# fryzjergda/DesiRNA

Hardware: AMD Instinct MI355X
Metric: replica-folds/sec (MFE+PF, L=200, R=64) (higher is better)
Workload: dtype int32 (MFE) + f64 (PF); 1 GPU; BASELINE configs[2]: Eterna100-V1 #69 target (L=200), R=64 uniform-random sequences per GPU, -sf Ed-Epf (MFE fill+traceback, PF inside, eval_structure); replicas_per_gpu=64, replicas_total=64, replicas_on_rank0=64, L=200, exchange_every=100, threads_per_workgroup=1024

## Files before the change

desirna_amd/csrc/engine.hip:

```cpp
#include <hip/hip_runtime.h>

#include <cstdio>
#include <cstdlib>
#include <cstring>
#include <ctime>
#include <algorithm>
#include <numeric>
#include <string>
#include <vector>

#include "../../include/desirna_amd.h"
#include "eval_structure.hpp"
#include "fold_mfe.hpp"
#include "fold_cofold.hpp"
#include "fold_cofold_lds.hpp"
#include "fold_self_dimer.hpp"
#include "fold_mfe_lds.hpp"
#include "fold_mfe_dual.hpp"
#include "fold_fused.hpp"
#include "fold_mfe_strip.hpp"
#include "fold_outside.hpp"
#include "fold_pf.hpp"
#include "fold_pf_lds.hpp"
#include "fold_pf_strip.hpp"
// ... 582 lines not shown
  else if (p.mfe_strips && ma.pk_rounds > 0 && R >= 16 * e->mfe_split && e->mfe_split > 1) {
    const int np = e->mfe_split, per = ((R + np - 1) / np + 7) / 8 * 8;
    const int pf_gate_round = pf_gate_env >= -1 ? pf_gate_env : (p.pf_strips && p.mfe_wgs >= e->cus && ma.pk_rounds >= 2) ? ma.pk_rounds - 1 : -1;
    for (int round = 0; round <= ma.pk_rounds; round++) {
      for (int part = 0, r0 = 0; r0 < R; part++, r0 += per) {
        const bool gate_here = round == pf_gate_round && p.want_pf && part == pf_gate_part;
        launch_mfe_strips_round(e, ma, std::min(per, R - r0), p.mfe_strips, r0, nullptr, r0, (part & 1) ? e->s_eval : e->s_mfe, round,
                                gate_here ? e->ev_gate : nullptr);
        if (gate_here) c.pf_gated = true;
      }
    }
    HIP_TRY(hipEventRecord(e->ev_mfe2, e->s_eval));
    HIP_TRY(hipStreamWaitEvent(e->s_mfe, e->ev_mfe2, 0));
  } else if (p.mfe_strips) launch_mfe_strips(e, ma, R, p.mfe_strips, 0, nullptr, e->s_mfe);
  else if (c.L <= MFE_FAST_NMAX) hipLaunchKernelGGL(mfe_lds_kernel<1024>, dim3(R), dim3(1024), 0, e->s_mfe, ma);
  else hipLaunchKernelGGL(mfe_kernel<1024>, dim3(R), dim3(1024), 0, e->s_mfe, ma);
  HIP_TRY(hipGetLastError());
  HIP_TRY(hipEventRecord(e->ev_m1, e->s_mfe));
  return DRNA_OK;
}
static int enqueue_eval(drna_engine* e, const FoldCall& c) {
  if (c.p.ev_in_pf) return DRNA_OK;
  HIP_TRY(hipEventRecord(e->ev_e0, c.s_ev));
  hipLaunchKernelGGL(eval_kernel, dim3(c.R * e->n_targets), dim3(WAVE), 0, c.s_ev, c.ev);
  HIP_TRY(hipGetLastError());
  HIP_TRY(hipEventRecord(e->ev_e1, c.s_ev));
  return DRNA_OK;
}
static int enqueue_folds(drna_engine* e, FoldCall& c) {
  const FoldPlan& p = c.p;
  e->last_fused = p.fused;
  e->last_wgs = p.mfe_wgs + p.pf_wgs;
  if (p.fused) {
    HIP_TRY(hipEventRecord(e->ev_m0, e->s_mfe));
    hipLaunchKernelGGL(score_fused_kernel<1024>, dim3(fused_grid(c.R)), dim3(1024), 0, e->s_mfe, c.ma, c.lk, c.pa, c.ev, c.R, e->d_clk);
    HIP_TRY(hipGetLastError());
    HIP_TRY(hipEventRecord(e->ev_m1, e->s_mfe));
    return DRNA_OK;
  }
  c.mfe_first = p.want_mfe && (!p.want_pf || e->timing[0] > e->timing[1]);
  c.s_ev = !(p.want_mfe && p.want_pf) ? e->s_eval : c.mfe_first ? e->s_pf : e->s_mfe;
  if (c.mfe_first) { const int rc = enqueue_mfe(e, c); if (rc != DRNA_OK) return rc; }
  if (p.want_ev && c.s_ev == e->s_pf) { const int rc = enqueue_eval(e, c); if (rc != DRNA_OK) return rc; }
  if (p.want_pf) { const int rc = enqueue_pf(e, c); if (rc != DRNA_OK) return rc; }
  if (p.want_ev && c.s_ev == e->s_mfe) { const int rc = enqueue_eval(e, c); if (rc != DRNA_OK) return rc; }
  if (p.want_mfe && !c.mfe_first) { const int rc = enqueue_mfe(e, c); if (rc != DRNA_OK) return rc; }
  if (p.want_ev && c.s_ev == e->s_eval) { const int rc = enqueue_eval(e, c); if (rc != DRNA_OK) return rc; }
  return DRNA_OK;
}

static int drain_folds(drna_engine* e, const FoldCall& c) {
  const FoldPlan& p = c.p;
  if (p.fused) {
    HIP_TRY(hipStreamSynchronize(e->s_mfe));
    float tot = 0.f;
    HIP_TRY(hipEventElapsedTime(&tot, e->ev_m0, e->ev_m1));
    const int grid = fused_grid(c.R);
    long long t0 = 0, end_mfe = 0, end_pf = 0;
    bool first = true;
    for (int b = 0; b < grid; b++) {
      int r, role;
      fused_block_role(b, r, role, grid);
      if (r >= c.R) continue;
      const long long s0 = e->h_clk[2 * b], s1 = e->h_clk[2 * b + 1];
      if (first || s0 < t0) t0 = s0;
      first = false;
      if (role <= ROLE_MFE_HELPER) { if (s1 > end_mfe) end_mfe = s1; } else if (s1 > end_pf) end_pf = s1;
    }
    e->timing[0] = (float)((end_mfe - t0) * 1e-5); e->timing[1] = (float)((end_pf - t0) * 1e-5);
    e->timing[2] = 0.f; e->timing[3] = tot;
    return DRNA_OK;
  }
  const bool ev_own = p.want_ev && !p.ev_in_pf;
  if (ev_own && c.s_ev == e->s_eval) HIP_TRY(hipStreamSynchronize(e->s_eval));
  if (c.mfe_first && p.want_pf) HIP_TRY(hipStreamSynchronize(e->s_pf));
  if (p.want_mfe) HIP_TRY(hipStreamSynchronize(e->s_mfe));
  if (!c.mfe_first && p.want_pf) HIP_TRY(hipStreamSynchronize(e->s_pf));
  e->timing[0] = e->timing[1] = e->timing[2] = e->timing[3] = 0.f;
  if (p.want_mfe) HIP_TRY(hipEventElapsedTime(&e->timing[0], e->ev_m0, e->ev_m1));
  if (p.want_pf) HIP_TRY(hipEventElapsedTime(&e->timing[1], e->ev_p0, e->ev_p1));
  if (ev_own) HIP_TRY(hipEventElapsedTime(&e->timing[2], e->ev_e0, e->ev_e1));
  hipEvent_t first = c.mfe_first ? e->ev_m0 : p.want_pf ? e->ev_p0 : e->ev_e0;
  float t = 0.f;
  if (p.want_mfe) { HIP_TRY(hipEventElapsedTime(&t, first, e->ev_m1)); e->timing[3] = std::max(e->timing[3], t); }
  if (p.want_pf) { HIP_TRY(hipEventElapsedTime(&t, first, e->ev_p1)); e->timing[3] = std::max(e->timing[3], t); }
  if (ev_own) { HIP_TRY(hipEventElapsedTime(&t, first, e->ev_e1)); e->timing[3] = std::max(e->timing[3], t); }
  return DRNA_OK;
}

static int score_batch_impl(drna_engine* e, int R, int L, const char* d_seqs, uint32_t flags, double* d_Epf, int32_t* d_Emfe,
                            char* d_mfe_ss, int32_t* d_Ed, int r_base) {
  HIP_TRY(hipSetDevice(e->device));
  FoldCall c{R, L, plan_uniform(e, R, L, flags)};
  const FoldPlan& p = c.p;
  { const int rc = prepare_folds(e, p, R); if (rc != DRNA_OK) return rc; }
  reset_status(e);
  e->cur_with_pf = p.want_pf;
  c.ev = p.want_ev ? eval_args(e, d_seqs, L, d_Ed) : EvalArgs{};
  c.ma = mfe_args(e, d_seqs, L, L + 2, p.want_pk ? 3 : 0, d_Emfe, d_mfe_ss);
  c.pa = pf_args(e, d_seqs, L, L + 2, d_Epf);
  if (p.pf_help) { c.pa.helper = e->helper_fault ? 2 : 1; c.pa.hflags = e->pflags.d; c.pa.hbase = epoch_base(e->pflags.epoch); }
  c.lk.flagA = e->dflags.d; c.lk.flagB = e->dflags.d;
  c.lk.xs = e->d_xs; c.lk.xa = e->d_xa_mfe; c.lk.xb = e->d_xb_mfe; c.lk.epoch = e->dflags.epoch;
// ... 1728 lines not shown
```

desirna_amd/csrc/fold_mfe.hpp:

```cpp
#pragma once
#include "fold_common.hpp"

namespace drna {

struct MfeArgs {
  const MfeTables* T;
  const Plan* plan;
  const int* hp_len;
  const char* seqs;
  int L;
  int ld;
  int pk_rounds;
  int32_t* ws;
  long long ws_stride;
  int32_t* Emfe;
  char* ss;
  int32_t* status;
  Ragged rg;
};

template <int NLEN>
struct MfeSmemCore {
  int stack[64];
  int mmH[128], mmI[128], mm1n[128], mm23[128], mmM[128], mmExt[128];
// ... 287 lines not shown
      }
      m = wave_min_i32(m);
      const int prev = sm.f5[j - 1];
      sm.f5[j] = prev < m ? prev : m;
    }
  }
  __syncthreads();
}


struct FmlGlobal {
  const int32_t* p;
  int ld;
  __device__ __forceinline__ int operator()(int d, int i) const { return p[d * ld + i]; }
};

template <class SM> struct TbStack {
  SM& sm;
  int sp = 0;
  __device__ __forceinline__ void init(int n) { sm.sec_i[0] = 1; sm.sec_j[0] = (short)n; sm.sec_ml[0] = 0; sp = 1; }
  __device__ __forceinline__ bool pop(int& i, int& j, int& ml) {
    if (sp == 0) return false;
    sp--;
    i = sm.sec_i[sp]; j = sm.sec_j[sp]; ml = sm.sec_ml[sp];
    return true;
  }
  __device__ __forceinline__ void push(int i, int j, int ml) { sm.sec_i[sp] = (short)i; sm.sec_j[sp] = (short)j; sm.sec_ml[sp] = (unsigned char)ml; sp++; }
  __device__ __forceinline__ void done_one() {}
  __device__ __forceinline__ void fail() {}
  __device__ __forceinline__ bool failed() const { return false; }
};
template <class SM> struct TbShared {
  SM& sm;
  __device__ __forceinline__ void init(int) {}
  __device__ __forceinline__ bool pop(int& i, int& j, int& ml) {
    int c = 0;
    if (lane_id() == 0) c = atomicAdd(&sm.tbq[0], 1);
    c = __builtin_amdgcn_readfirstlane(c);
    if (c > (int)(sizeof(sm.sec_ml) / sizeof(sm.sec_ml[0])) - 1) return false;
    for (;;) {
      const int m = __builtin_amdgcn_readfirstlane((int)*reinterpret_cast<volatile unsigned char*>(&sm.sec_ml[c]));
      if (m) {
        __builtin_amdgcn_fence(__ATOMIC_ACQUIRE, "workgroup");
        i = sm.sec_i[c]; j = sm.sec_j[c]; ml = m - 1;
        return true;
      }
      if (__builtin_amdgcn_readfirstlane(*reinterpret_cast<volatile int*>(&sm.tbq[3]))) return false;
      spin_pause();
    }
  }
  __device__ __forceinline__ void push(int i, int j, int ml) {
    if (lane_id() == 0) {
      atomicAdd(&sm.tbq[2], 1);
      const int c = atomicAdd(&sm.tbq[1], 1);
      if (c > (int)(sizeof(sm.sec_ml) / sizeof(sm.sec_ml[0])) - 1) { *reinterpret_cast<volatile int*>(&sm.tbq[3]) = 2; return; }
      sm.sec_i[c] = (short)i; sm.sec_j[c] = (short)j;
      __builtin_amdgcn_fence(__ATOMIC_RELEASE, "workgroup");
      *reinterpret_cast<volatile unsigned char*>(&sm.sec_ml[c]) = (unsigned char)(ml + 1);
    }
  }
  __device__ __forceinline__ void done_one() {
    if (lane_id() == 0 && atomicAdd(&sm.tbq[2], -1) == 1) *reinterpret_cast<volatile int*>(&sm.tbq[3]) = 1;
  }
  __device__ __forceinline__ void fail() { if (lane_id() == 0) *reinterpret_cast<volatile int*>(&sm.tbq[3]) = 2; }
  __device__ __forceinline__ bool failed() const { return *reinterpret_cast<volatile int*>(&sm.tbq[3]) == 2; }
};

template <class SM, class FMLACC, class QUEUE>
__device__ __forceinline__ bool mfe_traceback_q(SM& sm, const MfeArgs& A, const int32_t* __restrict__ Wc,
                                       const FMLACC FML, const int32_t* __restrict__ EXT, QUEUE Q) {
  const MfeTables& T = *A.T;
  const Plan& P = *A.plan;
  const int n = A.L, ld = A.ld, lane = lane_id();
  const int HALF = INF_DEV / 2;
  bool ok = true;
  constexpr int NRND = (NPLAN + WAVE - 1) / WAVE;
  int tb_shape[NRND], tb_L[NRND];
#pragma unroll
  for (int rnd = 0; rnd < NRND; rnd++) {
    const int k = rnd * WAVE + lane;
    tb_shape[rnd] = k < NPLAN ? P.tb_shape[k] : (PK_STACK << 16);
    tb_L[rnd] = k < NPLAN ? P.tb_L[k] : 0;
  }
  Q.init(n);
  auto sector = [&](int i, int j, const int ml) -> bool {
    bool have_pair = false;
    if (ml == 0) {
      if (j < TURN + 2) return true;
      int jj = -1;
      for (int base = j; base >= 1 && jj < 0; base -= WAVE) {
        const int x = base - lane;
        const bool hit = x >= 1 && sm.f5[x] != sm.f5[x - 1];
        const int fl = first_lane(__ballot(hit));
        if (fl >= 0) jj = base - fl;
      }
      if (jj < TURN + 2) return true;
      const int fij = sm.f5[jj];
      int u = -1;
      for (int base = jj - TURN - 1; base >= 1 && u < 0; base -= WAVE) {
        const int x = base - lane;
        bool hit = false;
        if (x >= 1) {
          const int e = EXT[jj * ld + x];
          hit = e < HALF && fij == e + sm.f5[x - 1];
        }
        const int fl = first_lane(__ballot(hit));
        if (fl >= 0) u = base - fl;
      }
      if (u < 0) return false;
      Q.push(1, (u - 1), 0);
      i = u; j = jj; have_pair = true;
    } else if (ml == 1) {
      for (;;) {
        const int jx = j - lane;
        bool stop = true;
        if (jx > i) {
          const int a = FML(jx - i, i), bq = (jx - 1 - i) >= 0 ? FML(jx - 1 - i, i) : INF_DEV;
          stop = !(a == bq + T.MLbase);
        }
        const int fl = first_lane(__ballot(stop));
        if (fl >= 0) { j -= fl; break; }
        j -= WAVE;
      }
      for (;;) {
        const int ix = i + lane;
        bool stop = true;
        if (ix < j) {
          const int a = FML(j - ix, ix), bq = FML(j - ix - 1, ix + 1);
          stop = !(a == bq + T.MLbase);
        }
        const int fl = first_lane(__ballot(stop));
        if (fl >= 0) { i += fl; break; }
        i += WAVE;
      }
      if (j < i + TURN + 1) return false;
      const int d = j - i;
      const int fij = FML(d, i);
      const int w = Wc[d * ld + i];
      const int cij = w >> 8;
      const int t = pair_type(sm.Sp[i], sm.Sp[j]);
      if (t && cij < HALF &&
          fij == cij + T.MLintern + (t > 2 ? T.TermAU : 0) + sm.mmM[t * 16 + sm.S[i - 1] * 4 + sm.S[j + 1]]) {
        have_pair = true;
      } else {
        int u = -1;
        for (int base = i + TURN + 1; base <= j - TURN - 2 && u < 0; base += WAVE) {
          const int x = base + lane;
          bool hit = false;
          if (x <= j - TURN - 2) hit = fij == FML(x - i, i) + FML(j - x - 1, x + 1);
          const int fl = first_lane(__ballot(hit));
          if (fl >= 0) u = base + fl;
        }
        if (u < 0) return false;
        Q.push(i, u, 1);
        Q.push((u + 1), j, 1);
      }
    } else {
      have_pair = true;
    }
    while (have_pair) {
      if (lane == 0) { sm.ssw[i - 1] = '('; sm.ssw[j - 1] = ')'; }
      const int d = j - i;
      const int t = pair_type(sm.Sp[i], sm.Sp[j]);
      const int w_in = d - 2 > TURN ? Wc[(d - 2) * ld + i + 1] : INF_DEV * 256;
      const int cij = Wc[d * ld + i] >> 8;
      if (cij == mfe_hairpin(sm, A, i, j, t)) break;
      const int si1 = sm.S[i + 1], sj1 = sm.S[j - 1];
      if ((w_in >> 8) < HALF && cij == (w_in >> 8) + mfe_intloop(sm, T, 0, 0, t, si1, sj1, w_in & 127)) {
        i++; j--;
        continue;
      }
      int found = -1;
      const int tij = t * 16 + si1 * 4 + sj1, tauI = t > 2 ? T.TermAU : 0;
#pragma unroll
      for (int rnd = 0; rnd < NRND; rnd++) {
        if (found >= 0) break;
        const int k = rnd * WAVE + lane;
        const int u1 = tb_shape[rnd] & 255, u2 = (tb_shape[rnd] >> 8) & 255, kind = tb_shape[rnd] >> 16;
        const int dp = d - 2 - u1 - u2;
        const bool live = k < NPLAN && dp > TURN;
        const int w = live ? Wc[dp * ld + i + 1 + u1] : INF_DEV * 256;
        const int cpq = w >> 8, info = w & 127, t2 = info >> 4, sq1 = (info >> 2) & 3, sp1 = info & 3;
        const int* mm = kind == PK_1XN ? sm.mm1n : kind == PK_INT23 ? sm.mm23 : sm.mmI;
        int en = mm[tij] + mm[info];
        const int e_stack = sm.stack[t * 8 + t2], e_11 = sm.int11[(t * 8 + t2) * 16 + si1 * 4 + sj1];
        en = kind == PK_STACK || kind == PK_BULGE1 ? e_stack : en;
        en = kind == PK_BULGEN ? tauI + (t2 > 2 ? T.TermAU : 0) : en;
        en = kind == PK_INT11 ? e_11 : en;
        if (kind == PK_INT21) en = T.int21[(t * 8 + t2) * 64 + si1 * 16 + sq1 * 4 + sj1];
        else if (kind == PK_INT12) en = T.int21[(t2 * 8 + t) * 64 + sq1 * 16 + si1 * 4 + sp1];
        else if (kind == PK_INT22) en = T.int22[(t * 8 + t2) * 256 + si1 * 64 + sp1 * 16 + sq1 * 4 + sj1];
        const bool hit = live && cpq < HALF && cij == cpq + en + tb_L[rnd];
        const int fl = first_lane(__ballot(hit));
        if (fl >= 0) found = rnd * WAVE + fl;
      }
      if (found >= 0) {
        i = i + 1 + P.tb_u1[found];
        j = j - 1 - P.tb_u2[found];
        continue;
      }
      const int e = cij - T.MLclosing - T.MLintern - (t > 2 ? T.TermAU : 0) -
                    sm.mmM[rtype_of(t) * 16 + sj1 * 4 + si1];
      int u = -1;
      for (int base = i + 2 + TURN; base < j - 2 - TURN && u < 0; base += WAVE) {
        const int x = base + lane;
        bool hit = false;
        if (x < j - 2 - TURN) hit = e == FML(x - i - 1, i + 1) + FML(j - 1 - x - 1, x + 1);
        const int fl = first_lane(__ballot(hit));
        if (fl >= 0) u = base + fl;
      }
      if (u < 0) return false;
      Q.push((i + 1), u, 1);
      Q.push((u + 1), (j - 1), 1);
      break;
    }
    return true;
  };
  int qi = 0, qj = 0, qml = 0;
  while (Q.pop(qi, qj, qml)) {
    if (!sector(qi, qj, qml)) { Q.fail(); ok = false; break; }
    Q.done_one();
  }
  return ok && !Q.failed();
}

template <class SM, class FMLACC>
__device__ inline bool mfe_traceback(SM& sm, const MfeArgs& A, const int32_t* __restrict__ Wc,
                                     const FMLACC FML, const int32_t* __restrict__ EXT) {
  return mfe_traceback_q(sm, A, Wc, FML, EXT, TbStack<SM>{sm});
}



template <int NT>
__global__ __launch_bounds__(NT) void mfe_kernel(MfeArgs A) {
  __shared__ MfeSmem sm;
  const int r = A.rg.seq_of(blockIdx.x);
  A.L = A.rg.len_of(r, A.L);
  const long long so = A.rg.off_of(r, A.L);
  const int n = A.L, ld = A.ld, tid = threadIdx.x;
  const MfeTables& T = *A.T;
  int32_t* base = A.ws + (long long)r * A.ws_stride;
  const long long tab = (long long)ld * ld;
  int32_t* Wc = base;
  int32_t* CI = base + tab;
  int32_t* FML = base + 2 * tab;
  int32_t* DML = base + 3 * tab;
  int32_t* EXT = base + 4 * tab;

  stage_energy_tables<NT>(sm, T, tid);
  load_sequence<NT>(sm, A.seqs + so, n, tid);
  if (sm.flag) {
    if (tid == 0) { A.status[r] = ST_BAD_CHAR; A.Emfe[r] = 0; }
    for (int k = tid; k < n; k += NT) A.ss[so + k] = '.';
    return;
  }
  pk_start<NT>(sm, n, tid);

  int status = ST_OK;
  for (int round = 0; round <= A.pk_rounds; round++) {
    for (int k = tid; k < n; k += NT) sm.ssw[k] = '.';
    mfe_fill<NT>(sm, A, Wc, CI, FML, DML, EXT);
// ... 17 lines not shown
```

desirna_amd/csrc/fold_mfe_lds.hpp:

```cpp
#pragma once
#include "fold_mfe.hpp"

namespace drna {

constexpr int MFE_FAST_NMAX = 200;
enum : int { E_ALL = 0, E_NEAR = 1, E_FAR = 2, E_COARSE = 3 };
constexpr int GSLOTS = 10;

template <int NT>
struct MfeFastSmem : MfeSmemCore<MFE_FAST_NMAX> {
  static constexpr int NW = NT / WAVE;
  static constexpr int RS = MFE_FAST_NMAX + 2;
  static constexpr int TRI = (MFE_FAST_NMAX - 4) * (MFE_FAST_NMAX - 3) / 2;
  static constexpr int NSLOT = 4 * WAVE;
  static constexpr int NL = MFE_FAST_NMAX + 8;
  int fml[TRI + 8];
  int wring[33 * RS];
  int ciring[32 * RS];
  int dml[4 * RS];
  int hpl[MFE_FAST_NMAX + 2];
  int rowoff[MFE_FAST_NMAX + 2];
  int accG[2][NSLOT], accI[2][NSLOT], accK[2][NSLOT];
  static constexpr int XT_STACK = 0, XT_INT11 = 64, XT_MM1N = 64 + 1024, XT_MM23 = 64 + 1024 + 128;
  int xtab[64 + 1024 + 128 + 128];
  int plist[2][NL];
  int xe[2][NL];
  int pcnt[2];
  int qhead[2];
  int eshape[128];
  int eshape_rows[128];
  int sync_fail;
  int tbq[4];
  int etab[2][128];
  int twc[32][2];
};

__device__ __forceinline__ int fml_off(int d, int n) { return (d - 4) * n - (d * (d - 1) / 2 - 6); }

template <int NT>
struct FmlLds {
  const MfeFastSmem<NT>* sm;
  int n;
  __device__ __forceinline__ int operator()(int d, int i) const {
    return d < TURN + 1 ? INF_DEV : sm->fml[fml_off(d, n) + i - 1];
  }
};

template <int NT>
__device__ __forceinline__ void mfe_f5_column(MfeFastSmem<NT>& sm, const int32_t* __restrict__ EXT, int ld, int j, int lane) {
  int m = INF_DEV;
  for (int i = lane + 1; i <= j - TURN - 1; i += WAVE) {
    const int x = EXT[j * ld + i];
    if (x < INF_DEV / 2) m = min(m, sm.f5[i - 1] + x);
  }
  m = wave_min_i32(m);
  const int prev = sm.f5[j - 1];
  sm.f5[j] = prev < m ? prev : m;
}

template <class SM>
__device__ __forceinline__ void mfe_prepare_etab(SM& sm, int d, int lane, int mode);
template <class SM>
__device__ __forceinline__ void mfe_prepare_tower_tab(SM& sm, int d, int tid, int ninio, int max_ninio) {
  constexpr int RS = SM::RS;
  const int par = d & 1;
// ... 744 lines not shown
  const long long so = A.rg.off_of(r, A.L);
  const int n = A.L, ld = A.ld, tid = threadIdx.x;
  const MfeTables& T = *A.T;
  int32_t* base = A.ws + (long long)r * A.ws_stride;
  const long long tab = (long long)ld * ld;
  int32_t* Wc = base;
  int32_t* EXT = base + 4 * tab;
  int32_t* PL = base + 3 * tab;
  int32_t* PLX = base + 1 * tab;

  for (int k = tid; k < 64; k += NT) sm.stack[k] = T.stack[k];
  for (int k = tid; k < 128; k += NT) {
    sm.mmH[k] = T.mmH[k]; sm.mmI[k] = T.mmI[k]; sm.mm1n[k] = T.mm1n[k];
    sm.mm23[k] = T.mm23[k]; sm.mmM[k] = T.mmM[k]; sm.mmExt[k] = T.mmExt[k];
  }
  for (int k = tid; k < 1024; k += NT) sm.int11[k] = T.int11[k];
  for (int k = tid; k < 32; k += NT) { sm.d5[k] = T.d5[k]; sm.d3[k] = T.d3[k]; }
  if (tid == 0) sm.sync_fail = 0;
  load_sequence<NT>(sm, A.seqs + so, n, tid);
  if (sm.flag) {
    if (tid == 0) { A.status[r] = ST_BAD_CHAR; A.Emfe[r] = 0; if (DUAL) st_agent(lk.flagA, dual_done(lk.epoch)); }
    for (int k = tid; k < n; k += NT) A.ss[so + k] = '.';
    return;
  }
  pk_start<NT>(sm, n, tid);

  int status = ST_OK;
  for (int round = 0; round <= A.pk_rounds; round++) {
    for (int k = tid; k < n; k += NT) sm.ssw[k] = '.';
    lk.base = dual_base(lk.epoch, round);
    mfe_fill_lds<NT, DUAL>(sm, A, Wc, EXT, PL, PLX, lk);
    if (DUAL && sm.sync_fail) { status = ST_SYNC; break; }
    constexpr int TB_WAVES = NT / WAVE < 8 ? NT / WAVE : 8;
    for (int k = tid; k < (int)(sizeof(sm.sec_ml) / sizeof(sm.sec_ml[0])); k += NT) sm.sec_ml[k] = 0;
    __syncthreads();
    if (tid == 0) {
      sm.sec_i[0] = 1; sm.sec_j[0] = (short)n; sm.sec_ml[0] = 1;
      sm.tbq[0] = 0; sm.tbq[1] = 1; sm.tbq[2] = 1; sm.tbq[3] = 0;
    }
    __syncthreads();
    if (wave_id() < TB_WAVES) (void)mfe_traceback_q(sm, A, Wc, FmlLds<NT>{&sm, n}, EXT, TbShared<MfeFastSmem<NT>>{sm});
    __syncthreads();
    if (tid == 0) {
      if (round == 0) A.Emfe[r] = sm.f5[n];
      sm.flag = sm.tbq[3] == 2 ? 1 : 0;
    }
    __syncthreads();
    if (sm.flag) { status = ST_TRACEBACK; break; }
    if (!pk_merge_round<NT>(sm, n, round)) break;
  }
  if (DUAL && tid == 0) st_agent(lk.flagA, dual_done(lk.epoch));
  for (int k = tid; k < n; k += NT) A.ss[so + k] = sm.sspk[k];
  if (tid == 0) A.status[r] = status;
}

template <int NT>
__global__ __launch_bounds__(NT) void mfe_lds_kernel(MfeArgs A) {
  __shared__ MfeFastSmem<NT> sm;
  const int r = A.rg.seq_of(blockIdx.x);
  mfe_lds_body<NT, false>(sm, A, r, DualLink{});
}

}
```

desirna_amd/csrc/fold_mfe_strip.hpp:

```cpp
#pragma once
#include "fold_mfe_lds.hpp"
#include <type_traits>

namespace drna {

constexpr int MSTRIP_REC = 96;

constexpr int MSTRIP_KU = 8;
#ifndef DRNA_MKT_W
#define DRNA_MKT_W 16
#endif
#ifndef DRNA_MKT_L
#define DRNA_MKT_L 4
#endif
constexpr int MKT_W = DRNA_MKT_W, MKT_L = DRNA_MKT_L;
constexpr int MKT_DEPTH = 2;
constexpr int MKT_BMIN = (44 + 2 * MKT_L + 15) / 16;
static_assert(MKT_W >= 1 && MKT_W <= 16 && MKT_L >= 3, "see tools/pkt_schedule.py");

template <int N>
__device__ __forceinline__ int row_bcast_i32(int v) { return __builtin_amdgcn_update_dpp(0, v, 0x150 + N, 0xF, 0xF, false); }

template <int NT>
struct MfeStripSmem {
// ... 618 lines not shown
  if (failed) {
    if (tid == 0) {
      if (has_down) st_agent(my_flag, lk.base + STRIP_FAIL);
      else { A.status[r] = ST_SYNC; Wc[0] = -1; }
    }
    return;
  }
  if (lk.clk && tid == 0) lk.clk[((long long)q * STRIP_MAXS + s) * 2 + 1] = wall_clock_100mhz();
  if (has_down) {
    if (tid == 0) st_agent(my_flag, lk.base + STRIP_DONE);
    return;
  }
  if (wave == 0) {
    for (int j = max(TURN + 2, n - 2); j <= n; j++) mstrip_f5_column(sm, rsE, ld, j, lane);
  }
  __syncthreads();
  for (int k = tid; k <= n; k += NT) Wc[ld + k] = sm.f5[k];
  if (tid == 0) Wc[0] = 2;
}

template <int NT, bool FARK>
__global__ __launch_bounds__(NT) void mfe_strip_kernel(MfeArgs A, StripLink lk, StripRec xr, int round) {
  __shared__ MfeStripSmem<NT> sm;
  const int b = blockIdx.x, per = 8 * (lk.S + lk.pad);
  const int grp = b / per, x = b - grp * per;
  const int q = grp * 8 + (x & 7), s = x >> 3;
  if (q >= lk.nseq || s >= lk.S) return;
  mfe_strip_body<NT, FARK>(sm, A, lk, xr, q, s, round);
}

constexpr int TRACE_WAVES = 8;
struct MfeTraceSmem : MfeSmemCore<STRIP_NMAX> {
  int tbq[4];
};

__device__ inline void mfe_strip_trace_body(MfeTraceSmem& sm, MfeArgs A, const int* idx, int q, int round, int r0 = 0) {
  constexpr int NT = TRACE_WAVES * WAVE;
  const int r = idx ? idx[q] : q + r0;
  A.L = A.rg.len_of(r, A.L);
  const long long so = A.rg.off_of(r, A.L);
  const int n = A.L, ld = A.ld, tid = threadIdx.x;
  const MfeTables& T = *A.T;
  int32_t* base = A.ws + (long long)r * A.ws_stride;
  const long long tab = (long long)ld * ld;
  int32_t* Wc = base;
  const int32_t* FML = base + 2 * tab;
  const int32_t* EXT = base + 4 * tab;
  const int state = Wc[0];
  if (round > 0 && state != 2) return;
  for (int k = tid; k < 64; k += NT) sm.stack[k] = T.stack[k];
  for (int k = tid; k < 128; k += NT) {
    sm.mmH[k] = T.mmH[k]; sm.mmI[k] = T.mmI[k]; sm.mm1n[k] = T.mm1n[k];
    sm.mm23[k] = T.mm23[k]; sm.mmM[k] = T.mmM[k]; sm.mmExt[k] = T.mmExt[k];
  }
  for (int k = tid; k < 1024; k += NT) sm.int11[k] = T.int11[k];
  for (int k = tid; k < 32; k += NT) { sm.d5[k] = T.d5[k]; sm.d3[k] = T.d3[k]; }
  for (int k = tid; k < n; k += NT) sm.ssw[k] = '.';
  for (int k = tid; k <= n; k += NT) sm.f5[k] = Wc[ld + k];
  for (int k = tid; k < (int)(sizeof(sm.sec_ml) / sizeof(sm.sec_ml[0])); k += NT) sm.sec_ml[k] = 0;
  load_sequence<NT>(sm, A.seqs + so, n, tid);
  if (sm.flag) {
    if (tid == 0) { A.status[r] = ST_BAD_CHAR; A.Emfe[r] = 0; Wc[0] = 0; }
    for (int k = tid; k < n; k += NT) A.ss[so + k] = '.';
    return;
  }
  if (state != 2) {
    if (tid == 0) { A.Emfe[r] = 0; Wc[0] = 0; }
    for (int k = tid; k < n; k += NT) A.ss[so + k] = '.';
    return;
  }
  for (int k = tid; k < n; k += NT) {
    const char prev = round > 0 ? A.ss[so + k] : '.';
    sm.sspk[k] = prev;
    sm.Sp[k + 1] = prev != '.' ? 4 : sm.S[k + 1];
  }
  if (tid == 0) {
    sm.Sp[0] = 4; sm.Sp[n + 1] = 4;
    sm.sec_i[0] = 1; sm.sec_j[0] = (short)n; sm.sec_ml[0] = 1;
    sm.tbq[0] = 0; sm.tbq[1] = 1; sm.tbq[2] = 1; sm.tbq[3] = 0;
  }
  __syncthreads();
  (void)mfe_traceback_q(sm, A, Wc, FmlGlobal{FML, ld}, EXT, TbShared<MfeTraceSmem>{sm});
  __syncthreads();
  if (sm.tbq[3] == 2) {
    if (tid == 0) { A.status[r] = ST_TRACEBACK; Wc[0] = 0; if (round == 0) A.Emfe[r] = sm.f5[n]; }
    for (int k = tid; k < n; k += NT) A.ss[so + k] = sm.sspk[k];
    return;
  }
  char op, cl;
  pk_brackets(round, op, cl);
  int any = 0;
  for (int k = tid; k < n; k += NT) {
    const char ch = sm.ssw[k];
    if (ch == '(') { sm.sspk[k] = op; any = 1; }
    else if (ch == ')') sm.sspk[k] = cl;
    A.ss[so + k] = sm.sspk[k];
  }
  if (any) sm.flag = 2;
  __syncthreads();
  if (tid == 0) {
    if (round == 0) A.Emfe[r] = sm.f5[n];
    A.status[r] = ST_OK;
    Wc[0] = ((round == 0 || sm.flag == 2) && round < A.pk_rounds) ? 1 : 0;
  }
}

__global__ __launch_bounds__(TRACE_WAVES * WAVE) void mfe_strip_trace_kernel(MfeArgs A, const int* idx, int nseq, int round, int r0) {
  __shared__ MfeTraceSmem sm;
  if ((int)blockIdx.x >= nseq) return;
  mfe_strip_trace_body(sm, A, idx, blockIdx.x, round, r0);
}

}
```

desirna_amd/csrc/tables.hpp:

```cpp
#pragma once
#include <cmath>
#include <cstdint>
#include <cstring>
#include <string>
#include <vector>

namespace drna {

constexpr int INF_REF = 10000000;
constexpr int INF_DEV = 1 << 22;
constexpr int TURN = 3;
constexpr int MAXLOOP = 30;
constexpr int NPLAN = 496;
constexpr int NPAIR_MAX = 256;
constexpr int MAX_SPECIAL = 64;

enum PlanKind : int {
  PK_STACK = 0, PK_BULGE1 = 1, PK_BULGEN = 2, PK_INT11 = 3, PK_INT21 = 4, PK_INT12 = 5,
  PK_1XN = 6, PK_INT22 = 7, PK_INT23 = 8, PK_GENERIC = 9, PK_NKINDS = 10
};

struct Plan {
  int u1[NPLAN], u2[NPLAN], kind[NPLAN];
  int L[NPLAN];
  double W[NPLAN];
  int seg[PK_NKINDS + 1];
  int tb_u1[NPLAN], tb_u2[NPLAN];
  int tb_shape[NPLAN], tb_L[NPLAN];
  int n_pair, n_quad;
  int pair_e[NPAIR_MAX], pair_n[NPAIR_MAX];
  int quad_e[NPAIR_MAX], quad_n[NPAIR_MAX];
};

struct MfeTables {
  int stack[64];
  int mmH[128], mmI[128], mm1n[128], mm23[128], mmM[128], mmExt[128];
  int d5[32], d3[32];
  int int11[1024];
  int int21[4096];
  int int22[16384];
  int bulge[31], interior[31];
  int ninio, max_ninio, MLbase, MLclosing, MLintern, TermAU;
  int n_tri, n_tetra, n_hexa;
  int tri_code[MAX_SPECIAL], tri_e[MAX_SPECIAL];
  int tetra_code[MAX_SPECIAL], tetra_e[MAX_SPECIAL];
  int hexa_code[MAX_SPECIAL], hexa_e[MAX_SPECIAL];
};

struct PfTables {
  double stack[64];
  double mmH[128], mmI[128], mm1n[128], mm23[128], mmM[128], mmExt[128];
  double d5[32], d3[32];
  double int11[1024];
  double int21[4096];
  double int22[16384];
  double bulge[31], interior[31], eninio[31];
  double MLbase, MLclosing, MLintern, TermAU;
  double kT, pf_scale;
  int n_tri, n_tetra, n_hexa;
  int tri_code[MAX_SPECIAL], tetra_code[MAX_SPECIAL], hexa_code[MAX_SPECIAL];
  double tri_w[MAX_SPECIAL], tetra_w[MAX_SPECIAL], hexa_w[MAX_SPECIAL];
// ... 181 lines not shown
        case PK_1XN:
          L = interior[nl + 1] + std::min(max_ninio, (nl - ns) * ninio);
          W = BF(interior[nl + 1]) * BF(std::min(max_ninio, (nl - ns) * ninio)); break;
        case PK_INT23:
          L = interior[5] + ninio; W = BF(interior[5]) * BF(std::min(max_ninio, ninio)); break;
        case PK_GENERIC:
          L = interior[s] + std::min(max_ninio, (nl - ns) * ninio);
          W = BF(interior[s]) * BF(std::min(max_ninio, (nl - ns) * ninio)); break;
        default: break;
      }
      P.L[e] = L;
      P.W[e] = W * std::pow(F.pf_scale, -(double)(s + 2));
      e++;
    }
  }
  P.seg[PK_NKINDS] = e;
  P.n_pair = P.n_quad = 0;
  for (int g = P.seg[PK_GENERIC]; g < NPLAN;) {
    int run = 1;
    while (g + run < NPLAN && P.u1[g + run] + P.u2[g + run] == P.u1[g] + P.u2[g] && P.u1[g + run] == P.u1[g] + run) run++;
    for (int x = 0; x < run; x += 2) { P.pair_e[P.n_pair] = g + x; P.pair_n[P.n_pair] = std::min(2, run - x); P.n_pair++; }
    for (int x = 0; x < run; x += 4) { P.quad_e[P.n_quad] = g + x; P.quad_n[P.n_quad] = std::min(4, run - x); P.n_quad++; }
    g += run;
  }
  e = 0;
  for (int u1 = 0; u1 <= MAXLOOP; u1++)
    for (int u2 = 0; u1 + u2 <= MAXLOOP; u2++) {
      const int k = kind_of(u1, u2), nl = std::max(u1, u2), ns = std::min(u1, u2);
      int L = 0;
      if (k == PK_BULGE1 || k == PK_BULGEN) L = M.bulge[nl];
      else if (k == PK_1XN) L = M.interior[nl + 1] + std::min(M.max_ninio, (nl - ns) * M.ninio);
      else if (k == PK_INT23) L = M.interior[5] + M.ninio;
      else if (k == PK_GENERIC) L = M.interior[nl + ns] + std::min(M.max_ninio, (nl - ns) * M.ninio);
      P.tb_u1[e] = u1; P.tb_u2[e] = u2; P.tb_shape[e] = u1 | (u2 << 8) | (k << 16); P.tb_L[e] = L; e++;
    }
  return "";
}

inline void size_tables(HostTables& T, int max_L) {
  const double kT = T.pf.kT;
  int N = (max_L > MAXLOOP + 4 ? max_L : MAXLOOP + 4) + 4;
  T.hp_len.assign(N, INF_DEV);
  T.hp_w.assign(N, 0.0);
  T.scale.assign(N, 1.0);
  T.eMLb.assign(N, 1.0);
  T.bulge_len.assign(N, INF_DEV);
  T.int_len.assign(N, INF_DEV);
  for (int k = 1; k < N; k++) {
    T.scale[k] = T.scale[k - 1] / T.pf.pf_scale;
    T.eMLb[k] = T.eMLb[k - 1] * T.pf.MLbase / T.pf.pf_scale;
  }
  for (int u = 0; u < N; u++) {
    if (u <= 30) {
      T.hp_len[u] = T.hairpin[u];
      T.hp_w[u] = T.ehairpin[u];
      T.bulge_len[u] = T.mfe.bulge[u];
      T.int_len[u] = T.mfe.interior[u];
    } else {
      int ext = (int)(T.lxc * std::log(u / 30.0));
      T.hp_len[u] = T.hairpin[30] + ext;
      T.hp_w[u] = T.ehairpin[30] * std::exp(-(T.lxc * std::log(u / 30.0)) * 10.0 / kT);
      T.bulge_len[u] = T.mfe.bulge[30] + ext;
      T.int_len[u] = T.mfe.interior[30] + ext;
    }
    if (u + 2 < N) T.hp_w[u] *= T.scale[u + 2];
  }
}

// ... 2 lines not shown
```

Measured before the change: 151,700 replica-folds/s.

## Streamline MFE traceback queue, table loads, and interior-loop search

The shared traceback work queue now packs each sector's (i,j,ml) into a single int written and read with LDS atomics, replacing separate arrays with fences. The traceback plan shape and L tables are packed into one padded array and loaded with buffer loads. Hairpin energy is computed inline, with special-hairpin lookup done as a wave-wide ballot and hairpin lengths read from LDS. The interior-loop search batches W loads and int21/int22 lookups in groups before the ballot. The fused path drops its event records and derives total time from clock stamps, which removes host-side event overhead but changes what timing[3] reports.

```diff
diff --git a/desirna_amd/csrc/engine.hip b/desirna_amd/csrc/engine.hip
--- a/desirna_amd/csrc/engine.hip
+++ b/desirna_amd/csrc/engine.hip
@@ -638,10 +638,8 @@
   e->last_fused = p.fused;
   e->last_wgs = p.mfe_wgs + p.pf_wgs;
   if (p.fused) {
-    HIP_TRY(hipEventRecord(e->ev_m0, e->s_mfe));
     hipLaunchKernelGGL(score_fused_kernel<1024>, dim3(fused_grid(c.R)), dim3(1024), 0, e->s_mfe, c.ma, c.lk, c.pa, c.ev, c.R, e->d_clk);
     HIP_TRY(hipGetLastError());
-    HIP_TRY(hipEventRecord(e->ev_m1, e->s_mfe));
     return DRNA_OK;
   }
   c.mfe_first = p.want_mfe && (!p.want_pf || e->timing[0] > e->timing[1]);
@@ -659,8 +657,6 @@
   const FoldPlan& p = c.p;
   if (p.fused) {
     HIP_TRY(hipStreamSynchronize(e->s_mfe));
-    float tot = 0.f;
-    HIP_TRY(hipEventElapsedTime(&tot, e->ev_m0, e->ev_m1));
     const int grid = fused_grid(c.R);
     long long t0 = 0, end_mfe = 0, end_pf = 0;
     bool first = true;
@@ -674,7 +670,7 @@
       if (role <= ROLE_MFE_HELPER) { if (s1 > end_mfe) end_mfe = s1; } else if (s1 > end_pf) end_pf = s1;
     }
     e->timing[0] = (float)((end_mfe - t0) * 1e-5); e->timing[1] = (float)((end_pf - t0) * 1e-5);
-    e->timing[2] = 0.f; e->timing[3] = tot;
+    e->timing[2] = 0.f; e->timing[3] = std::max(e->timing[0], e->timing[1]);
     return DRNA_OK;
   }
   const bool ev_own = p.want_ev && !p.ev_in_pf;
diff --git a/desirna_amd/csrc/fold_mfe.hpp b/desirna_amd/csrc/fold_mfe.hpp
--- a/desirna_amd/csrc/fold_mfe.hpp
+++ b/desirna_amd/csrc/fold_mfe.hpp
@@ -343,20 +343,24 @@
 };
 template <class SM> struct TbShared {
   SM& sm;
+  static constexpr int CAP = (int)(sizeof(SM::tbw) / sizeof(int));
+  static __host__ __device__ constexpr int word(int i, int j, int ml) { return i | (j << 11) | ((ml + 1) << 22); }
+  __device__ __forceinline__ int peek(int* p) const {
+    int v = 0;
+    if (lane_id() == 0) v = atomicAdd(p, 0);
+    return __builtin_amdgcn_readfirstlane(v);
+  }
   __device__ __forceinline__ void init(int) {}
   __device__ __forceinline__ bool pop(int& i, int& j, int& ml) {
-    int c = 0;
-    if (lane_id() == 0) c = atomicAdd(&sm.tbq[0], 1);
-    c = __builtin_amdgcn_readfirstlane(c);
-    if (c > (int)(sizeof(sm.sec_ml) / sizeof(sm.sec_ml[0])) - 1) return false;
+    const int c = queue_pop(&sm.tbq[0], lane_id());
+    if (c > CAP - 1) return false;
     for (;;) {
-      const int m = __builtin_amdgcn_readfirstlane((int)*reinterpret_cast<volatile unsigned char*>(&sm.sec_ml[c]));
-      if (m) {
-        __builtin_amdgcn_fence(__ATOMIC_ACQUIRE, "workgroup");
-        i = sm.sec_i[c]; j = sm.sec_j[c]; ml = m - 1;
+      const int w = peek(&sm.tbw[c]);
+      if (w) {
+        i = w & 2047; j = (w >> 11) & 2047; ml = (w >> 22) - 1;
         return true;
       }
-      if (__builtin_amdgcn_readfirstlane(*reinterpret_cast<volatile int*>(&sm.tbq[3]))) return false;
+      if (peek(&sm.tbq[3])) return false;
       spin_pause();
     }
   }
@@ -364,35 +368,71 @@
     if (lane_id() == 0) {
       atomicAdd(&sm.tbq[2], 1);
       const int c = atomicAdd(&sm.tbq[1], 1);
-      if (c > (int)(sizeof(sm.sec_ml) / sizeof(sm.sec_ml[0])) - 1) { *reinterpret_cast<volatile int*>(&sm.tbq[3]) = 2; return; }
-      sm.sec_i[c] = (short)i; sm.sec_j[c] = (short)j;
-      __builtin_amdgcn_fence(__ATOMIC_RELEASE, "workgroup");
-      *reinterpret_cast<volatile unsigned char*>(&sm.sec_ml[c]) = (unsigned char)(ml + 1);
+      if (c > CAP - 1) { atomicAdd(&sm.tbq[3], 2); return; }
+      atomicAdd(&sm.tbw[c], word(i, j, ml));
     }
   }
   __device__ __forceinline__ void done_one() {
-    if (lane_id() == 0 && atomicAdd(&sm.tbq[2], -1) == 1) *reinterpret_cast<volatile int*>(&sm.tbq[3]) = 1;
-  }
-  __device__ __forceinline__ void fail() { if (lane_id() == 0) *reinterpret_cast<volatile int*>(&sm.tbq[3]) = 2; }
-  __device__ __forceinline__ bool failed() const { return *reinterpret_cast<volatile int*>(&sm.tbq[3]) == 2; }
-};
-
-template <class SM, class FMLACC, class QUEUE>
+    if (lane_id() == 0 && atomicAdd(&sm.tbq[2], -1) == 1) atomicAdd(&sm.tbq[3], 1);
+  }
+  __device__ __forceinline__ void fail() { if (lane_id() == 0) atomicAdd(&sm.tbq[3], 2); }
+  __device__ __forceinline__ bool failed() const { return peek(&sm.tbq[3]) >= 2; }
+};
+
+struct HplGlobal {
+  const int* p;
+  __device__ __forceinline__ int operator()(int u) const { return p[u]; }
+};
+template <class SM> struct HplLds {
+  const SM* sm;
+  __device__ __forceinline__ int operator()(int u) const { return sm->hpl[u]; }
+};
+
+__device__ __forceinline__ bool tb_special_hairpin(const int* codes, const int* es, int cnt, int code, int lane, int& e) {
+  static_assert(MAX_SPECIAL <= WAVE, "one table entry per lane");
+  const int c = lane < cnt ? codes[lane] : -1, v = lane < cnt ? es[lane] : 0;
+  const int fl = first_lane(__ballot(c == code));
+  if (fl < 0) return false;
+  e = __builtin_amdgcn_readlane(v, fl);
+  return true;
+}
+
+template <class SM, class FMLACC, class HPLACC, class QUEUE>
 __device__ __forceinline__ bool mfe_traceback_q(SM& sm, const MfeArgs& A, const int32_t* __restrict__ Wc,
-                                       const FMLACC FML, const int32_t* __restrict__ EXT, QUEUE Q) {
+                                       const FMLACC FML, const HPLACC HPL, const int32_t* __restrict__ EXT, QUEUE Q) {
   const MfeTables& T = *A.T;
   const Plan& P = *A.plan;
   const int n = A.L, ld = A.ld, lane = lane_id();
   const int HALF = INF_DEV / 2;
   bool ok = true;
-  constexpr int NRND = (NPLAN + WAVE - 1) / WAVE;
+  constexpr int NRND = NPLAN_TB / WAVE;
   int tb_shape[NRND], tb_L[NRND];
-#pragma unroll
-  for (int rnd = 0; rnd < NRND; rnd++) {
-    const int k = rnd * WAVE + lane;
-    tb_shape[rnd] = k < NPLAN ? P.tb_shape[k] : (PK_STACK << 16);
-    tb_L[rnd] = k < NPLAN ? P.tb_L[k] : 0;
-  }
+  {
+    const auto rsP = __builtin_amdgcn_make_buffer_rsrc((void*)&P.tb_pack[0][0], (short)0, (int)sizeof(P.tb_pack), 0x00020000);
+    const int voff = as_vector(lane) * 8;
+#pragma unroll
+    for (int rnd = 0; rnd < NRND; rnd++) {
+      const auto v = __builtin_amdgcn_raw_buffer_load_b64(rsP, voff, rnd * WAVE * 8, 0);
+      tb_shape[rnd] = (int)v[0]; tb_L[rnd] = (int)v[1];
+    }
+  }
+  const int cMLbase = keep_i32(T.MLbase), cMLintern = keep_i32(T.MLintern), cMLclosing = keep_i32(T.MLclosing), cTermAU = keep_i32(T.TermAU);
+  const int n_tri = keep_i32(T.n_tri), n_tetra = keep_i32(T.n_tetra), n_hexa = keep_i32(T.n_hexa);
+  auto hairpin = [&](int i, int j, int t) -> int {
+    const int u = j - i - 1, e = HPL(u);
+    if (u == 3 || u == 4 || u == 6) {
+      int code = 0;
+      for (int k = 0; k < u + 2; k++) code |= sm.S[i + k] << (2 * k);
+      int es = 0;
+      if (u == 3) {
+        if (n_tri && tb_special_hairpin(T.tri_code, T.tri_e, n_tri, code, lane, es)) return es;
+        return e + (t > 2 ? cTermAU : 0);
+      }
+      if (u == 4 ? (n_tetra && tb_special_hairpin(T.tetra_code, T.tetra_e, n_tetra, code, lane, es))
+                 : (n_hexa && tb_special_hairpin(T.hexa_code, T.hexa_e, n_hexa, code, lane, es))) return es;
+    }
+    return e + sm.mmH[t * 16 + sm.S[i + 1] * 4 + sm.S[j - 1]];
+  };
   Q.init(n);
   auto sector = [&](int i, int j, const int ml) -> bool {
     bool have_pair = false;
@@ -427,7 +467,7 @@
         bool stop = true;
         if (jx > i) {
           const int a = FML(jx - i, i), bq = (jx - 1 - i) >= 0 ? FML(jx - 1 - i, i) : INF_DEV;
-          stop = !(a == bq + T.MLbase);
+          stop = !(a == bq + cMLbase);
         }
         const int fl = first_lane(__ballot(stop));
         if (fl >= 0) { j -= fl; break; }
@@ -438,7 +478,7 @@
         bool stop = true;
         if (ix < j) {
           const int a = FML(j - ix, ix), bq = FML(j - ix - 1, ix + 1);
-          stop = !(a == bq + T.MLbase);
+          stop = !(a == bq + cMLbase);
         }
         const int fl = first_lane(__ballot(stop));
         if (fl >= 0) { i += fl; break; }
@@ -451,7 +491,7 @@
       const int cij = w >> 8;
       const int t = pair_type(sm.Sp[i], sm.Sp[j]);
       if (t && cij < HALF &&
-          fij == cij + T.MLintern + (t > 2 ? T.TermAU : 0) + sm.mmM[t * 16 + sm.S[i - 1] * 4 + sm.S[j + 1]]) {
+          fij == cij + cMLintern + (t > 2 ? cTermAU : 0) + sm.mmM[t * 16 + sm.S[i - 1] * 4 + sm.S[j + 1]]) {
         have_pair = true;
       } else {
         int u = -1;
@@ -475,42 +515,59 @@
       const int t = pair_type(sm.Sp[i], sm.Sp[j]);
       const int w_in = d - 2 > TURN ? Wc[(d - 2) * ld + i + 1] : INF_DEV * 256;
       const int cij = Wc[d * ld + i] >> 8;
-      if (cij == mfe_hairpin(sm, A, i, j, t)) break;
+      if (cij == hairpin(i, j, t)) break;
       const int si1 = sm.S[i + 1], sj1 = sm.S[j - 1];
       if ((w_in >> 8) < HALF && cij == (w_in >> 8) + mfe_intloop(sm, T, 0, 0, t, si1, sj1, w_in & 127)) {
         i++; j--;
         continue;
       }
-      int found = -1;
-      const int tij = t * 16 + si1 * 4 + sj1, tauI = t > 2 ? T.TermAU : 0;
-#pragma unroll
-      for (int rnd = 0; rnd < NRND; rnd++) {
-        if (found >= 0) break;
-        const int k = rnd * WAVE + lane;
-        const int u1 = tb_shape[rnd] & 255, u2 = (tb_shape[rnd] >> 8) & 255, kind = tb_shape[rnd] >> 16;
-        const int dp = d - 2 - u1 - u2;
-        const bool live = k < NPLAN && dp > TURN;
-        const int w = live ? Wc[dp * ld + i + 1 + u1] : INF_DEV * 256;
-        const int cpq = w >> 8, info = w & 127, t2 = info >> 4, sq1 = (info >> 2) & 3, sp1 = info & 3;
-        const int* mm = kind == PK_1XN ? sm.mm1n : kind == PK_INT23 ? sm.mm23 : sm.mmI;
-        int en = mm[tij] + mm[info];
-        const int e_stack = sm.stack[t * 8 + t2], e_11 = sm.int11[(t * 8 + t2) * 16 + si1 * 4 + sj1];
-        en = kind == PK_STACK || kind == PK_BULGE1 ? e_stack : en;
-        en = kind == PK_BULGEN ? tauI + (t2 > 2 ? T.TermAU : 0) : en;
-        en = kind == PK_INT11 ? e_11 : en;
-        if (kind == PK_INT21) en = T.int21[(t * 8 + t2) * 64 + si1 * 16 + sq1 * 4 + sj1];
-        else if (kind == PK_INT12) en = T.int21[(t2 * 8 + t) * 64 + sq1 * 16 + si1 * 4 + sp1];
-        else if (kind == PK_INT22) en = T.int22[(t * 8 + t2) * 256 + si1 * 64 + sp1 * 16 + sq1 * 4 + sj1];
-        const bool hit = live && cpq < HALF && cij == cpq + en + tb_L[rnd];
-        const int fl = first_lane(__ballot(hit));
-        if (fl >= 0) found = rnd * WAVE + fl;
-      }
-      if (found >= 0) {
-        i = i + 1 + P.tb_u1[found];
-        j = j - 1 - P.tb_u2[found];
+      const int tij = t * 16 + si1 * 4 + sj1, tauI = t > 2 ? cTermAU : 0;
+      constexpr int TB_GRP[] = {0, 2, NRND};
+      int wq[NRND], eq[NRND];
+      int fshape = -1;
+#pragma unroll
+      for (int g = 0; g + 1 < (int)(sizeof(TB_GRP) / sizeof(int)); g++) {
+        if (fshape >= 0) break;
+#pragma unroll
+        for (int rnd = TB_GRP[g]; rnd < TB_GRP[g + 1]; rnd++) {
+          const int u1 = tb_shape[rnd] & 255, u2 = (tb_shape[rnd] >> 8) & 255;
+          const int dp = d - 2 - u1 - u2;
+          const bool live = rnd * WAVE + lane < NPLAN && dp > TURN;
+          wq[rnd] = live ? Wc[dp * ld + i + 1 + u1] : INF_DEV * 256;
+        }
+#pragma unroll
+        for (int rnd = TB_GRP[g]; rnd < TB_GRP[g + 1]; rnd++) {
+          const int kind = tb_shape[rnd] >> 16;
+          const int info = wq[rnd] & 127, t2 = info >> 4, sq1 = (info >> 2) & 3, sp1 = info & 3;
+          int en = 0;
+          if (kind == PK_INT21) en = T.int21[(t * 8 + t2) * 64 + si1 * 16 + sq1 * 4 + sj1];
+          else if (kind == PK_INT12) en = T.int21[(t2 * 8 + t) * 64 + sq1 * 16 + si1 * 4 + sp1];
+          else if (kind == PK_INT22) en = T.int22[(t * 8 + t2) * 256 + si1 * 64 + sp1 * 16 + sq1 * 4 + sj1];
+          eq[rnd] = en;
+        }
+#pragma unroll
+        for (int rnd = TB_GRP[g]; rnd < TB_GRP[g + 1]; rnd++) {
+          if (fshape >= 0) break;
+          const int kind = tb_shape[rnd] >> 16;
+          const int cpq = wq[rnd] >> 8, info = wq[rnd] & 127, t2 = info >> 4;
+          const int* mm = kind == PK_1XN ? sm.mm1n : kind == PK_INT23 ? sm.mm23 : sm.mmI;
+          int en = mm[tij] + mm[info];
+          const int e_stack = sm.stack[t * 8 + t2], e_11 = sm.int11[(t * 8 + t2) * 16 + si1 * 4 + sj1];
+          en = kind == PK_STACK || kind == PK_BULGE1 ? e_stack : en;
+          en = kind == PK_BULGEN ? tauI + (t2 > 2 ? cTermAU : 0) : en;
+          en = kind == PK_INT11 ? e_11 : en;
+          en = kind == PK_INT21 || kind == PK_INT12 || kind == PK_INT22 ? eq[rnd] : en;
+          const bool hit = cpq < HALF && cij == cpq + en + tb_L[rnd];
+          const int fl = first_lane(__ballot(hit));
+          if (fl >= 0) fshape = __builtin_amdgcn_readlane(tb_shape[rnd], fl);
+        }
+      }
+      if (fshape >= 0) {
+        i = i + 1 + (fshape & 255);
+        j = j - 1 - ((fshape >> 8) & 255);
         continue;
       }
-      const int e = cij - T.MLclosing - T.MLintern - (t > 2 ? T.TermAU : 0) -
+      const int e = cij - cMLclosing - cMLintern - (t > 2 ? cTermAU : 0) -
                     sm.mmM[rtype_of(t) * 16 + sj1 * 4 + si1];
       int u = -1;
       for (int base = i + 2 + TURN; base < j - 2 - TURN && u < 0; base += WAVE) {
@@ -538,7 +595,7 @@
 template <class SM, class FMLACC>
 __device__ inline bool mfe_traceback(SM& sm, const MfeArgs& A, const int32_t* __restrict__ Wc,
                                      const FMLACC FML, const int32_t* __restrict__ EXT) {
-  return mfe_traceback_q(sm, A, Wc, FML, EXT, TbStack<SM>{sm});
+  return mfe_traceback_q(sm, A, Wc, FML, HplGlobal{A.hp_len}, EXT, TbStack<SM>{sm});
 }
 
 
diff --git a/desirna_amd/csrc/fold_mfe_lds.hpp b/desirna_amd/csrc/fold_mfe_lds.hpp
--- a/desirna_amd/csrc/fold_mfe_lds.hpp
+++ b/desirna_amd/csrc/fold_mfe_lds.hpp
@@ -31,6 +31,7 @@
   int eshape_rows[128];
   int sync_fail;
   int tbq[4];
+  int tbw[MFE_FAST_NMAX + 2];
   int etab[2][128];
   int twc[32][2];
 };
@@ -841,18 +842,15 @@
     mfe_fill_lds<NT, DUAL>(sm, A, Wc, EXT, PL, PLX, lk);
     if (DUAL && sm.sync_fail) { status = ST_SYNC; break; }
     constexpr int TB_WAVES = NT / WAVE < 8 ? NT / WAVE : 8;
-    for (int k = tid; k < (int)(sizeof(sm.sec_ml) / sizeof(sm.sec_ml[0])); k += NT) sm.sec_ml[k] = 0;
+    for (int k = tid; k < TbShared<MfeFastSmem<NT>>::CAP; k += NT) sm.tbw[k] = k ? 0 : TbShared<MfeFastSmem<NT>>::word(1, n, 0);
+    if (tid == 0) { sm.tbq[0] = 0; sm.tbq[1] = 1; sm.tbq[2] = 1; sm.tbq[3] = 0; }
     __syncthreads();
-    if (tid == 0) {
-      sm.sec_i[0] = 1; sm.sec_j[0] = (short)n; sm.sec_ml[0] = 1;
-      sm.tbq[0] = 0; sm.tbq[1] = 1; sm.tbq[2] = 1; sm.tbq[3] = 0;
-    }
-    __syncthreads();
-    if (wave_id() < TB_WAVES) (void)mfe_traceback_q(sm, A, Wc, FmlLds<NT>{&sm, n}, EXT, TbShared<MfeFastSmem<NT>>{sm});
+    if (wave_id() < TB_WAVES)
+      (void)mfe_traceback_q(sm, A, Wc, FmlLds<NT>{&sm, n}, HplLds<MfeFastSmem<NT>>{&sm}, EXT, TbShared<MfeFastSmem<NT>>{sm});
     __syncthreads();
     if (tid == 0) {
       if (round == 0) A.Emfe[r] = sm.f5[n];
-      sm.flag = sm.tbq[3] == 2 ? 1 : 0;
+      sm.flag = sm.tbq[3] >= 2 ? 1 : 0;
     }
     __syncthreads();
     if (sm.flag) { status = ST_TRACEBACK; break; }
diff --git a/desirna_amd/csrc/fold_mfe_strip.hpp b/desirna_amd/csrc/fold_mfe_strip.hpp
--- a/desirna_amd/csrc/fold_mfe_strip.hpp
+++ b/desirna_amd/csrc/fold_mfe_strip.hpp
@@ -674,6 +674,7 @@
 constexpr int TRACE_WAVES = 8;
 struct MfeTraceSmem : MfeSmemCore<STRIP_NMAX> {
   int tbq[4];
+  int tbw[STRIP_NMAX + 2];
 };
 
 __device__ inline void mfe_strip_trace_body(MfeTraceSmem& sm, MfeArgs A, const int* idx, int q, int round, int r0 = 0) {
@@ -699,7 +700,7 @@
   for (int k = tid; k < 32; k += NT) { sm.d5[k] = T.d5[k]; sm.d3[k] = T.d3[k]; }
   for (int k = tid; k < n; k += NT) sm.ssw[k] = '.';
   for (int k = tid; k <= n; k += NT) sm.f5[k] = Wc[ld + k];
-  for (int k = tid; k < (int)(sizeof(sm.sec_ml) / sizeof(sm.sec_ml[0])); k += NT) sm.sec_ml[k] = 0;
+  for (int k = tid; k < TbShared<MfeTraceSmem>::CAP; k += NT) sm.tbw[k] = 0;
   load_sequence<NT>(sm, A.seqs + so, n, tid);
   if (sm.flag) {
     if (tid == 0) { A.status[r] = ST_BAD_CHAR; A.Emfe[r] = 0; Wc[0] = 0; }
@@ -718,13 +719,13 @@
   }
   if (tid == 0) {
     sm.Sp[0] = 4; sm.Sp[n + 1] = 4;
-    sm.sec_i[0] = 1; sm.sec_j[0] = (short)n; sm.sec_ml[0] = 1;
+    sm.tbw[0] = TbShared<MfeTraceSmem>::word(1, n, 0);
     sm.tbq[0] = 0; sm.tbq[1] = 1; sm.tbq[2] = 1; sm.tbq[3] = 0;
   }
   __syncthreads();
-  (void)mfe_traceback_q(sm, A, Wc, FmlGlobal{FML, ld}, EXT, TbShared<MfeTraceSmem>{sm});
+  (void)mfe_traceback_q(sm, A, Wc, FmlGlobal{FML, ld}, HplGlobal{A.hp_len}, EXT, TbShared<MfeTraceSmem>{sm});
   __syncthreads();
-  if (sm.tbq[3] == 2) {
+  if (sm.tbq[3] >= 2) {
     if (tid == 0) { A.status[r] = ST_TRACEBACK; Wc[0] = 0; if (round == 0) A.Emfe[r] = sm.f5[n]; }
     for (int k = tid; k < n; k += NT) A.ss[so + k] = sm.sspk[k];
     return;
diff --git a/desirna_amd/csrc/tables.hpp b/desirna_amd/csrc/tables.hpp
--- a/desirna_amd/csrc/tables.hpp
+++ b/desirna_amd/csrc/tables.hpp
@@ -12,6 +12,7 @@
 constexpr int TURN = 3;
 constexpr int MAXLOOP = 30;
 constexpr int NPLAN = 496;
+constexpr int NPLAN_TB = (NPLAN + 63) / 64 * 64;
 constexpr int NPAIR_MAX = 256;
 constexpr int MAX_SPECIAL = 64;
 
@@ -26,7 +27,7 @@
   double W[NPLAN];
   int seg[PK_NKINDS + 1];
   int tb_u1[NPLAN], tb_u2[NPLAN];
-  int tb_shape[NPLAN], tb_L[NPLAN];
+  int tb_pack[NPLAN_TB][2];
   int n_pair, n_quad;
   int pair_e[NPAIR_MAX], pair_n[NPAIR_MAX];
   int quad_e[NPAIR_MAX], quad_n[NPAIR_MAX];
@@ -274,8 +275,9 @@
       else if (k == PK_1XN) L = M.interior[nl + 1] + std::min(M.max_ninio, (nl - ns) * M.ninio);
       else if (k == PK_INT23) L = M.interior[5] + M.ninio;
       else if (k == PK_GENERIC) L = M.interior[nl + ns] + std::min(M.max_ninio, (nl - ns) * M.ninio);
-      P.tb_u1[e] = u1; P.tb_u2[e] = u2; P.tb_shape[e] = u1 | (u2 << 8) | (k << 16); P.tb_L[e] = L; e++;
-    }
+      P.tb_u1[e] = u1; P.tb_u2[e] = u2; P.tb_pack[e][0] = u1 | (u2 << 8) | (k << 16); P.tb_pack[e][1] = L; e++;
+    }
+  for (; e < NPLAN_TB; e++) { P.tb_pack[e][0] = 255 | (255 << 8) | (PK_STACK << 16); P.tb_pack[e][1] = 0; }
   return "";
 }
 
```

Result: faster. 154,200 replica-folds/s (median of 6 runs) (+1.7%).
